# acids-ircam/RAVE

Hardware: AMD Instinct MI355X
Metric: audio samples/sec/GPU (RAVE v2 training step, 44.1 kHz, n_signal=65536) (higher is better)
Workload: dtype f32; 1 GPU; v2 config, batch 32 mono 44.1 kHz n_signal=65536, VAE-phase training step per GPU (--phase vae); global_batch=32, parallelism=dp1, phase=vae

## Files before the change

include/rave_hip.h:

```cpp
#ifndef RAVE_HIP_H
#define RAVE_HIP_H

#include <stddef.h>
#include <stdint.h>

#ifdef __cplusplus
extern "C" {
#endif

#define RH_VERSION 100

#define RH_OK 0
#define RH_ERR_INVALID (-1)
#define RH_ERR_UNSUPPORTED (-2)
#define RH_ERR_WORKSPACE (-3)

typedef void* rh_stream_t;

enum rh_act {
    RH_ACT_NONE = 0,
    RH_ACT_LEAKY = 1,
    RH_ACT_SNAKE = 2
};

// ... 21 lines not shown
const char* rh_last_error(void);



int rh_weight_norm_fwd_f32(const float* v, const float* g, int64_t rows, int64_t cols, float* w,
                           float* norms, rh_stream_t stream);
int rh_weight_norm_bwd_f32(const float* dw, const float* v, const float* g, const float* norms,
                           int64_t rows, int64_t cols, float* dv, float* dg, rh_stream_t stream);
typedef struct rh_wn_bwd_item {
    const float* dw;
    const float* v;
    const float* g;
    const float* norms;
    float* dv;
    float* dg;
    int64_t rows;
    int64_t cols;
} rh_wn_bwd_item;
int rh_weight_norm_bwd_batched_f32(const rh_wn_bwd_item* items, int32_t n_items, rh_stream_t stream);
typedef struct rh_reduce_item {
    const float* part;
    float* out;
    int64_t n;
    int32_t Z;
    int32_t reserved;
} rh_reduce_item;
int rh_defer_reduce(rh_reduce_item* item);
int rh_reduce_partials_batched_f32(const rh_reduce_item* items, int32_t n_items, rh_stream_t stream);

int64_t rh_conv1d_packed_floats(const rh_conv1d_desc* d, int which);
int rh_conv1d_pack_f32(const rh_conv1d_desc* d, const float* w, float* wp_fwd, float* wp_bwd,
                       rh_stream_t stream);

int rh_conv1d_pack_wn_f32(const rh_conv1d_desc* d, const float* v, const float* g, float* norms,
                          float* scale, float* wp_fwd, float* wp_bwd, rh_stream_t stream);

int64_t rh_prep_item_bytes(void);
int64_t rh_prep_array_bytes(int32_t n);
int rh_prep_fill_item(const rh_conv1d_desc* d, const float* v, const float* g, float* norms, float* scale,
                      float* wp_fwd, float* wp_bwd, void* item_host);
int rh_prep_link(void* items_host, int32_t n, int64_t* total_rows, int64_t* total_blocks);
int rh_prep_run_f32(const void* items_dev, int32_t n, int64_t total_rows, int64_t total_blocks, rh_stream_t stream);


int rh_conv1d_fwd_f32(const rh_conv1d_desc* d, const float* x, const float* wp_fwd,
                      const float* bias, const float* snake_alpha, const float* residual,
                      float* y, void* workspace, int64_t workspace_bytes, rh_stream_t stream);
int64_t rh_conv1d_fwd_workspace_bytes(const rh_conv1d_desc* d);
int64_t rh_conv1d_bwd_data_workspace_bytes(const rh_conv1d_desc* d);
int rh_conv1d_kernel_family(const rh_conv1d_desc* d, int which, int has_bias, int has_add);
int rh_residual_unit_fused(const rh_conv1d_desc* d3, const rh_conv1d_desc* d1);
int rh_residual_unit_fwd_f32(const rh_conv1d_desc* d3, const rh_conv1d_desc* d1, const float* x, const float* wp3_fwd,
                             const float* wp1_fwd, float* h, float* y, rh_stream_t stream);

int rh_x6_uses_ranges(void);
int rh_x6_range_words(void);
int rh_x6_set_ranges(const uint32_t* in_a, const uint32_t* in_b, uint32_t* out, uint32_t* out2);
int rh_amax_f32(const float* x, int64_t n, uint32_t* slot, rh_stream_t stream);

int rh_conv1d_plan_info(const rh_conv1d_desc* d, int which, int has_bias, int has_add, int32_t* out8);
int rh_conv1d_bwd_weight_kernel_family(const rh_conv1d_desc* d);

int rh_conv1d_bwd_data_f32(const rh_conv1d_desc* d, const float* dy, const float* wp_bwd,
                           const float* x, const float* snake_alpha, const float* add, float* dx,
                           void* workspace, int64_t workspace_bytes, rh_stream_t stream);

int64_t rh_conv1d_workspace_bytes(const rh_conv1d_desc* d);
int rh_conv1d_bwd_weight_f32(const rh_conv1d_desc* d, const float* dy, const float* x,
                             const float* snake_alpha, float* dw, float* dbias, void* workspace,
                             int64_t workspace_bytes, rh_stream_t stream);
int rh_conv1d_bwd_weight_wn_f32(const rh_conv1d_desc* d, const float* dy, const float* x, const float* snake_alpha,
                                const float* v, const float* g, const float* norms, float* dw_scratch, float* dv,
                                float* dg, float* dbias, void* workspace, int64_t workspace_bytes, rh_stream_t stream);
int64_t rh_conv1d_bwd_weight_wn_fused_launches(void);


int rh_pqmf_analysis_fwd_f32(const float* x, const float* w, int32_t rows, int32_t t_len,
                             int32_t n_band, int32_t kernel, int32_t pad_left, int32_t n_frames,
                             float* y, rh_stream_t stream);
int rh_pqmf_analysis_bwd_f32(const float* dy, const float* w, int32_t rows, int32_t t_len,
                             int32_t n_band, int32_t kernel, int32_t pad_left, int32_t n_frames,
                             float* dx, rh_stream_t stream);
int rh_pqmf_synthesis_fwd_f32(const float* y, const float* w, int32_t rows, int32_t n_frames,
                              int32_t n_band, int32_t kernel, int32_t pad_left, int32_t n_out,
                              float* x, rh_stream_t stream);
int rh_pqmf_synthesis_bwd_f32(const float* dx, const float* w, int32_t rows, int32_t n_frames,
                              int32_t n_band, int32_t kernel, int32_t pad_left, int32_t n_out,
                              float* dy, rh_stream_t stream);

int rh_pqmf_fold_k1_f32(const float* in, const float* tab, int32_t rows, int32_t t_len, int32_t n_frames, int32_t o0,
                        float scale, float* out, rh_stream_t stream);
int rh_pqmf_fold_k2_f32(const float* in, const float* tab, int32_t rows, int32_t n_frames, int32_t n_out, int32_t dp,
                        float scale, float* out, rh_stream_t stream);


int rh_amp_tanh_fwd_f32(const float* x, int32_t batch, int32_t c, int32_t l, float* y,
                        rh_stream_t stream);
int rh_amp_tanh_bwd_f32(const float* dy, const float* x, int32_t batch, int32_t c, int32_t l,
                        float* dx, rh_stream_t stream);
int rh_act_fwd_f32(const float* x, const float* snake_alpha, int32_t act, float slope,
                   int32_t batch, int32_t c, int32_t l, float* y, rh_stream_t stream);
int64_t rh_snake_bwd_workspace_bytes(int32_t batch, int32_t c);
int rh_snake_bwd_f32(const float* dy, const float* x, const float* alpha, int32_t batch, int32_t c,
                     int32_t l, float* dx, float* dalpha, void* workspace, int64_t workspace_bytes,
                     rh_stream_t stream);
int rh_act_bwd_f32(const float* dy, const float* y, int32_t act, float slope, int64_t n, float* g, rh_stream_t stream);
// ... 132 lines not shown
```

rave_amd/_lib.py:

```python
from __future__ import annotations

import ctypes as C
import os

import torch

_HERE = os.path.dirname(os.path.abspath(__file__))
LIB_PATH = os.environ.get("RAVE_HIP_LIB") or os.path.join(_HERE, "librave_hip.so")

ACT_NONE, ACT_LEAKY, ACT_SNAKE = 0, 1, 2


class ConvDesc(C.Structure):
    _fields_ = [
        ("batch", C.c_int32), ("c_in", C.c_int32), ("c_out", C.c_int32),
        ("l_in", C.c_int32), ("l_out", C.c_int32), ("kernel", C.c_int32),
        ("stride", C.c_int32), ("dilation", C.c_int32), ("pad_left", C.c_int32),
        ("transposed", C.c_int32), ("groups", C.c_int32), ("inner", C.c_int32),
        ("in_valid", C.c_int32), ("act", C.c_int32), ("act_slope", C.c_float),
        ("out_act", C.c_int32), ("out_slope", C.c_float),
    ]


class AdamItem(C.Structure):
# ... 3 lines not shown
class WnBwdItem(C.Structure):
    _fields_ = [("dw", C.c_void_p), ("v", C.c_void_p), ("g", C.c_void_p), ("norms", C.c_void_p), ("dv", C.c_void_p),
                ("dg", C.c_void_p), ("rows", C.c_int64), ("cols", C.c_int64)]


class ReduceItem(C.Structure):
    _fields_ = [("part", C.c_void_p), ("out", C.c_void_p), ("n", C.c_int64), ("Z", C.c_int32), ("reserved", C.c_int32)]


class LossItem(C.Structure):
    _fields_ = [("value", C.c_void_p), ("w1_dev", C.c_void_p), ("w1", C.c_float), ("w2", C.c_float)]


class FmItem(C.Structure):
    _fields_ = [("f", C.c_void_p), ("df", C.c_void_p), ("half", C.c_int64), ("w", C.c_float)]


class Conv2dDesc(C.Structure):
    _fields_ = [(n, C.c_int32) for n in (
        "batch", "c_in", "c_out", "h_in", "w_in", "h_out", "w_out", "kh", "kw", "sh", "sw", "dh", "dw", "ph", "pw",
        "act")] + [("act_slope", C.c_float)]


def _load() -> C.CDLL:
    if not os.path.exists(LIB_PATH):
        raise RuntimeError(
            f"rave_amd: {LIB_PATH} not found. Build it with `python -m rave_amd.build` "
            "(or __graft_entry__.build()). There is no CPU / PyTorch fallback for the HIP hot path.")
    lib = C.CDLL(LIB_PATH)
    P, I32, I64, F = C.c_void_p, C.c_int32, C.c_int64, C.c_float
    D = C.POINTER(ConvDesc)
    D2 = C.POINTER(Conv2dDesc)
    sig = {
        "rh_version": ([], C.c_int),
        "rh_last_error": ([], C.c_char_p),
        "rh_weight_norm_fwd_f32": ([P, P, I64, I64, P, P, P], C.c_int),
        "rh_weight_norm_bwd_f32": ([P, P, P, P, I64, I64, P, P, P], C.c_int),
        "rh_weight_norm_bwd_batched_f32": ([C.POINTER(WnBwdItem), I32, P], C.c_int),
        "rh_defer_reduce": ([C.POINTER(ReduceItem)], C.c_int),
        "rh_reduce_partials_batched_f32": ([C.POINTER(ReduceItem), I32, P], C.c_int),
        "rh_conv1d_packed_floats": ([D, C.c_int], I64),
        "rh_conv1d_pack_f32": ([D, P, P, P, P], C.c_int),
        "rh_conv1d_pack_wn_f32": ([D, P, P, P, P, P, P, P], C.c_int),
        "rh_prep_item_bytes": ([], I64),
        "rh_prep_array_bytes": ([I32], I64),
        "rh_prep_fill_item": ([D, P, P, P, P, P, P, P], C.c_int),
        "rh_prep_link": ([P, I32, C.POINTER(I64), C.POINTER(I64)], C.c_int),
        "rh_prep_run_f32": ([P, I32, I64, I64, P], C.c_int),
        "rh_conv1d_fwd_f32": ([D, P, P, P, P, P, P, P, I64, P], C.c_int),
        "rh_conv1d_bwd_data_f32": ([D, P, P, P, P, P, P, P, I64, P], C.c_int),
        "rh_conv1d_kernel_family": ([D, C.c_int, C.c_int, C.c_int], C.c_int),
        "rh_conv1d_bwd_weight_kernel_family": ([D], C.c_int),
        "rh_residual_unit_fused": ([D, D], C.c_int),
        "rh_residual_unit_fwd_f32": ([D, D, P, P, P, P, P, P], C.c_int),
        "rh_conv1d_plan_info": ([D, C.c_int, C.c_int, C.c_int, C.POINTER(C.c_int32)], C.c_int),
        "rh_conv1d_fwd_workspace_bytes": ([D], I64),
        "rh_conv1d_bwd_data_workspace_bytes": ([D], I64),
        "rh_conv1d_workspace_bytes": ([D], I64),
        "rh_conv1d_bwd_weight_f32": ([D, P, P, P, P, P, P, I64, P], C.c_int),
        "rh_conv1d_bwd_weight_wn_f32": ([D, P, P, P, P, P, P, P, P, P, P, P, I64, P], C.c_int),
        "rh_conv1d_bwd_weight_wn_fused_launches": ([], I64),
        "rh_conv2d_packed_floats": ([D2, C.c_int], I64),
        "rh_conv2d_pack_f32": ([D2, P, P, P, P], C.c_int),
        "rh_conv2d_fwd_f32": ([D2, P, P, P, P, P], C.c_int),
        "rh_conv2d_bwd_data_f32": ([D2, P, P, P, P, P], C.c_int),
        "rh_conv2d_workspace_bytes": ([D2], I64),
        "rh_conv2d_plan_info": ([D2, I32, C.POINTER(I64)], C.c_int),
        "rh_conv2d_bwd_weight_kernel_family": ([D2], C.c_int),
        "rh_conv2d_bwd_weight_f32": ([D2, P, P, P, P, P, P, I64, P], C.c_int),
        "rh_feed_batch_i16_f32": ([P, P, P, P, I32, I32, I32, P, P], C.c_int),
        "rh_vq_loss_partials": ([I64], I64),
        "rh_vq_assign_f32": ([P, P, I64, I32, I32, P, P, P, P, P], C.c_int),
        "rh_vq_assign_workspace_bytes": ([I64, I32, I32], I64),
        "rh_vq_assign_ws_f32": ([P, P, I64, I32, I32, P, P, P, P, P, I64, P], C.c_int),
        "rh_vq_ema_update_f32": ([P, P, I64, I32, I32, F, F, P, P, P, P], C.c_int),
        "rh_pqmf_analysis_fwd_f32": ([P, P, I32, I32, I32, I32, I32, I32, P, P], C.c_int),
        "rh_pqmf_analysis_bwd_f32": ([P, P, I32, I32, I32, I32, I32, I32, P, P], C.c_int),
        "rh_pqmf_synthesis_fwd_f32": ([P, P, I32, I32, I32, I32, I32, I32, P, P], C.c_int),
        "rh_pqmf_synthesis_bwd_f32": ([P, P, I32, I32, I32, I32, I32, I32, P, P], C.c_int),
        "rh_pqmf_fold_k1_f32": ([P, P, I32, I32, I32, I32, F, P, P], C.c_int),
        "rh_pqmf_fold_k2_f32": ([P, P, I32, I32, I32, I32, F, P, P], C.c_int),
        "rh_amp_tanh_fwd_f32": ([P, I32, I32, I32, P, P], C.c_int),
        "rh_amp_tanh_bwd_f32": ([P, P, I32, I32, I32, P, P], C.c_int),
        "rh_act_fwd_f32": ([P, P, I32, F, I32, I32, I32, P, P], C.c_int),
        "rh_act_bwd_f32": ([P, P, I32, F, I64, P, P], C.c_int),
        "rh_act_bwd_bias_workspace_bytes": ([I32], I64),
        "rh_act_bwd_bias_f32": ([P, P, I32, F, I32, I32, I64, P, P, P, I64, P], C.c_int),
        "rh_snake_bwd_workspace_bytes": ([I32, I32], I64),
        "rh_snake_bwd_f32": ([P, P, P, I32, I32, I32, P, P, P, I64, P], C.c_int),
        "rh_stft_frame_fwd_f32": ([P, P, I64, I32, I32, I32, I32, P, P], C.c_int),
        "rh_stft_frame_bwd_f32": ([P, P, I64, I32, I32, I32, I32, P, P], C.c_int),
        "rh_stft_frame_bwd_acc_f32": ([P, P, I64, I32, I32, I32, I32, P, I32, P], C.c_int),
        "rh_spectral_total_f32": ([P, P, I32, P, P], C.c_int),
        "rh_feature_matching_workspace_bytes": ([C.POINTER(FmItem), I32], I64),
        "rh_feature_matching_fwd_f32": ([C.POINTER(FmItem), I32, I32, P, I64, P, P, P], C.c_int),
        "rh_feature_matching_bwd_f32": ([C.POINTER(FmItem), I32, I32, P, P, P], C.c_int),
        "rh_reparam_workspace_bytes": ([], I64),
        "rh_reparam_fwd_f32": ([P, P, I32, I32, I32, P, P, P, I64, P], C.c_int),
        "rh_reparam_bwd_f32": ([P, P, P, P, I32, I32, I32, P, P], C.c_int),
        "rh_loss_combine_fwd_f32": ([C.POINTER(LossItem), I32, P, P, P], C.c_int),
        "rh_loss_combine_bwd_f32": ([C.POINTER(LossItem), I32, P, P, P], C.c_int),
        "rh_adam_step_f32": ([C.POINTER(AdamItem), I32, P, F, F, F, P, P], C.c_int),
        "rh_x6_uses_ranges": ([], C.c_int),
        "rh_x6_range_words": ([], C.c_int),
        "rh_x6_set_ranges": ([P, P, P, P], C.c_int),
        "rh_amax_f32": ([P, I64, P, P], C.c_int),
# ... 42 lines not shown
```

rave_amd/build.py:

```python
from __future__ import annotations

import hashlib
import os
import subprocess
import sys
from concurrent.futures import ThreadPoolExecutor

HERE = os.path.dirname(os.path.abspath(__file__))
CSRC = os.path.join(HERE, "csrc")
OBJ = os.path.join(HERE, "_obj")
LIB = os.path.join(HERE, "librave_hip.so")
SOURCES = ["api.cpp", "pqmf.hip", "pqmf_fold.hip", "pqmf_fold2.hip", "conv_igemm.hip", "conv_igemm_dma.hip", "conv_x6.hip", "conv_x6_i1_121.hip", "conv_x6_i1_221.hip", "conv_x6_i1_321.hip", "conv_x6_i1_122.hip", "conv_x6_i1_222.hip", "conv_x6_i1_322.hip", "conv_x6_i1_211.hip", "conv_x6_i1_311.hip", "conv_x6_i1_212.hip", "conv_x6_i1_312.hip", "conv_x6_i2_121.hip", "conv_x6_i2_221.hip", "conv_x6_i2_321.hip", "conv_x6_i2_122.hip", "conv_x6_i2_222.hip", "conv_x6_i2_322.hip", "conv_x6_i2_211.hip", "conv_x6_i2_311.hip", "conv_x6_i2_212.hip", "conv_x6_i2_312.hip", "conv_x6_i4_121.hip", "conv_x6_i4_221.hip", "conv_x6_i4_321.hip", "conv_x6_i4_122.hip", "conv_x6_i4_222.hip", "conv_x6_i4_322.hip", "conv_x6_i4_211.hip", "conv_x6_i4_311.hip", "conv_x6_i4_212.hip", "conv_x6_i4_312.hip", "unit_x6.hip", "conv_host.hip", "conv_wgrad.hip", "conv_wgrad_x6.hip", "conv_smallc.hip", "conv2d.hip", "conv2d_x6.hip", "conv2d_smallm.hip", "conv2d_smallc.hip", "wgrad2d_x6.hip", "vq.hip", "feed.hip", "misc.hip", "stft_loss.hip", "adam.hip", "feature_match.hip"]
HEADERS = ["common.hpp", "conv_params.hpp", "conv2d_x6.hpp", "conv_x6_kernel.inc", os.path.join("..", "..", "include", "rave_hip.h")]
FLAGS = ["--offload-arch=gfx950", "-O3", "-std=c++17", "-fPIC", "-Wall", "-Wno-unused-function"]


def _hipcc() -> str:
    for c in (os.environ.get("HIPCC"), "/opt/rocm/bin/hipcc", "hipcc"):
        if c and (os.path.isabs(c) and os.path.exists(c) or not os.path.isabs(c)):
            return c
    raise RuntimeError("hipcc not found")


def _digest(paths) -> str:
    h = hashlib.sha256()
    for p in paths:
        with open(p, "rb") as f:
            h.update(f.read())
    h.update(" ".join(FLAGS).encode())
    return h.hexdigest()


def build(force: bool = False, verbose: bool = False, _variants: bool = True) -> str:
    os.makedirs(OBJ, exist_ok=True)
    hdrs = [os.path.join(CSRC, h) for h in HEADERS]
    hip = _hipcc()
    jobs = []
    objs = []
    for s in SOURCES:
        src = os.path.join(CSRC, s)
        obj = os.path.join(OBJ, s + ".o")
        stamp = obj + ".sha"
        dig = _digest([src] + hdrs)
        objs.append(obj)
        if not force and os.path.exists(obj) and os.path.exists(stamp) and open(stamp).read() == dig:
            continue
        lang = ["-x", "hip"] if s.endswith(".hip") or s.endswith(".cpp") else []
        jobs.append((s, [hip] + FLAGS + lang + ["-c", src, "-o", obj], stamp, dig))

    def run(job):
        name, cmd, stamp, dig = job
        r = subprocess.run(cmd, capture_output=True, text=True)
        if r.returncode != 0:
            raise RuntimeError(f"hipcc failed for {name}:\n{r.stdout}\n{r.stderr}")
        if verbose and r.stderr.strip():
            print(r.stderr, file=sys.stderr)
        with open(stamp, "w") as f:
            f.write(dig)
        return name

    if jobs:
        with ThreadPoolExecutor(max_workers=min(len(jobs), os.cpu_count() or 4)) as ex:
            list(ex.map(run, jobs))
    if jobs or not os.path.exists(LIB) or force:
        cmd = [hip, "--offload-arch=gfx950", "-shared", "-fPIC", "-o", LIB] + objs
        r = subprocess.run(cmd, capture_output=True, text=True)
# ... 91 lines not shown
```

rave_amd/csrc/unit_x6.hip:

```cpp
#include <cstdlib>
#include <mutex>
#include <type_traits>
#include "conv_params.hpp"
#include "conv_x6_kernel.inc"

bool rh_conv_x6_plan_fixed(ConvP& p, int tm, int tn, int wm, size_t* lds, dim3* grid);

namespace {

struct UnitP {
    ConvP c;
    const unsigned* wq1;
    unsigned wq1_bytes;
    float slope2;
    float* h_out;
    const unsigned* w1_range;
    unsigned* h_range;
};

template <int TM, int TN>
__global__ __launch_bounds__(256, 2) void unit_x6_kernel(const UnitP u) {
    const ConvP& p = u.c;
    constexpr int WN = 4;
    constexpr int BM = 32 * TM;
    constexpr int A_UNITS = 2 * kX6P * BM;
    constexpr int NAL = (A_UNITS + 255) / 256;
    constexpr int NQ = WN * TN == 8 ? 3 : 2;
    extern __shared__ __attribute__((aligned(16))) unsigned char smem_raw[];
    u32x4* const a_st = reinterpret_cast<u32x4*>(smem_raw);
    u32x4* const b_st = a_st + 2 * A_UNITS;

    const int tid = threadIdx.x, lane = tid & 63;
    const int wn = __builtin_amdgcn_readfirstlane(tid >> 6);
    const int j = lane & 31, g = lane >> 5;

    const int tap0 = p.ph_tap0[0];
    const int minoff = p.ph_minoff[0];
    const int nu = p.ph_ntaps[0];
    const int bt = blockIdx.x / p.tiles_per_b;
    const int nt = blockIdx.x - bt * p.tiles_per_b;
    const int b0 = bt * p.nb;
    const int n0 = nt * p.bnl;
    const int pitch = p.pitch, P = p.x6_P;
    const float slope1 = p.in_act == RH_ACT_LEAKY ? p.in_slope : 1.f;

    const auto in_rsrc = __builtin_amdgcn_make_buffer_rsrc(const_cast<float*>(p.in), 0, p.in_bytes, 0x00020000);
    const auto w_rsrc = __builtin_amdgcn_make_buffer_rsrc(const_cast<unsigned*>(p.wq), 0, p.wq_bytes, 0x00020000);
#if RH_X6_F16
    int inv_x, inv_w3, inv_h, inv_w1;
    const unsigned xmax = rh_range_max(p.in_range);
    const float xsc = __uint_as_float(rh_x6_scale_bits(xmax, &inv_x));
    (void)rh_x6_scale_bits(p.w_range[0], &inv_w3);
    const float osc1 = __uint_as_float(rh_x6_unscale_bits(inv_w3, inv_x));
    const float hbound = __uint_as_float(xmax) * __uint_as_float(p.w_range[1]);
    const unsigned hsc_bits = rh_x6_scale_bits(__float_as_uint(hbound), &inv_h);
    (void)rh_x6_scale_bits(u.w1_range[0], &inv_w1);
    const float osc2 = __uint_as_float(rh_x6_unscale_bits(inv_w1, inv_h));
    const float h2sc = __uint_as_float(rh_x6_unscale_bits(inv_w3 + (int)(hsc_bits >> 23) - 127, inv_x));
#else
    const float xsc = 1.f, osc1 = 1.f, osc2 = 1.f, h2sc = 1.f;
#endif

    int bpos[TN];
#pragma unroll
    for (int tn = 0; tn < TN; ++tn) {
        const int col = (wn * TN + tn) * 32 + j;
        const int bl = col >> p.bnl_shift;
        const int nl = col & (p.bnl - 1);
        const int n = min(n0 + nl, p.ncols - 1);
        bpos[tn] = g * kX6P * P + bl * pitch + (n - n0);
    }
// ... 194 lines not shown
            for (int r = 0; r < 16; ++r) acc2[tm][0][r] = 0.f;
#pragma unroll
        for (int b = 0; b < 2 * TM; ++b) {
            const int tmh = b >> 1, hf = b & 1;
            float v[8];
#pragma unroll
            for (int i = 0; i < 8; ++i) v[i] = acc[tmh][tn][8 * hf + i];
            u32x4 pk[kX6P];
            split8(v, u.slope2, h2sc, pk);
            rh_x6_frag bfr2[kX6P], afr2[TM][kX6P];
#pragma unroll
            for (int s3 = 0; s3 < kX6P; ++s3) {
                auto r0 = __builtin_amdgcn_permlane32_swap(pk[s3][0], pk[s3][2], false, false);
                auto r1 = __builtin_amdgcn_permlane32_swap(pk[s3][1], pk[s3][3], false, false);
                u32x4 f;
                f[0] = r0[0]; f[2] = r0[1]; f[1] = r1[0]; f[3] = r1[1];
                bfr2[s3] = __builtin_bit_cast(rh_x6_frag, f);
            }
            const u32x4* al = w1s + (b * 2 * kX6P + g * kX6P) * BM + j;
#pragma unroll
            for (int tm = 0; tm < TM; ++tm)
#pragma unroll
                for (int s3 = 0; s3 < kX6P; ++s3) afr2[tm][s3] = __builtin_bit_cast(rh_x6_frag, al[s3 * BM + tm * 32]);
#pragma unroll
            for (int q = 0; q < RH_X6_NPROD; ++q)
#pragma unroll
                for (int tm = 0; tm < TM; ++tm)
                    acc2[tm][0] = RH_X6_MFMA(afr2[tm][SA[q]], bfr2[SB[q]], acc2[tm][0]);
        }
        const unsigned cb1[1] = {cb[tn]};
        x6_store_tile<4, TM, 1>(acc2, cb1, 0, g, p.M, full, p.out_row, y_r, none_r, x_r, none_r, 1.f, 0.f, osc2, ymax);
    }
    if (RH_X6_F16 && (p.out_range || u.h_range)) {
        __syncthreads();
        float* red = reinterpret_cast<float*>(smem_raw);
        if (p.out_range) rh_range_publish(p.out_range, ymax, blockIdx.x, red);
        if (u.h_range) rh_range_publish(u.h_range, hmax_all, blockIdx.x + 5u, red + 4);
    }
}

bool unit_enabled() {
    const char* e = getenv("RH_UNIT_FUSED");
    if (e && atoi(e) == 0) return false;
    const char* x6 = getenv("RH_CONV_X6");
    return !(x6 && atoi(x6) == 0);
}

bool unit_shape_ok(const rh_conv1d_desc* d3, const rh_conv1d_desc* d1) {
    if (!d3 || !d1) return false;
    const int C = d3->c_in;
    auto act_ok = [](const rh_conv1d_desc* d) {
        return d->act == RH_ACT_NONE || (d->act == RH_ACT_LEAKY && d->act_slope >= 0.f && d->act_slope <= 1.f);
    };
    return (C == 32 || C == 64 || C == 96) && d3->c_out == C && d1->c_in == C && d1->c_out == C && !d3->transposed &&
           !d1->transposed && d3->stride == 1 && d1->stride == 1 && d3->inner == 1 && d1->inner == 1 && d3->groups == 1 &&
           d1->groups == 1 && d1->kernel == 1 && d1->dilation == 1 && d1->pad_left == 0 && d3->in_valid == 0 &&
           d1->in_valid == 0 && d3->out_act == RH_ACT_NONE && d1->out_act == RH_ACT_NONE && act_ok(d3) && act_ok(d1) &&
           d3->batch > 0 && d3->batch == d1->batch && d3->l_in > 0 && d3->l_out == d3->l_in && d1->l_in == d3->l_in &&
           d1->l_out == d3->l_in;
}

int fill_unit(const rh_conv1d_desc* d3, const rh_conv1d_desc* d1, UnitP* u, size_t* lds, dim3* grid) {
    ConvP& p = u->c;
    if (int e = rh_conv_fill_fwd(d3, &p)) return e;
    ConvP p1{};
    if (int e = rh_conv_fill_fwd(d1, &p1)) return e;
    if (p.x6_mode != 1 || p1.x6_mode != 1 || p.nphase != 1) return RH_ERR_UNSUPPORTED;
    const int tm = p.M / 32;
    if (!rh_conv_x6_plan_fixed(p, tm, 2, 1, lds, grid)) return RH_ERR_UNSUPPORTED;
    const size_t w1_bytes = (size_t)(p.M / 16) * 2 * kX6P * p.M * 16;
    if (w1_bytes > *lds) *lds = w1_bytes;
    if (*lds > 160 * 1024 || (unsigned long long)p1.wq_bytes < w1_bytes) return RH_ERR_UNSUPPORTED;
    u->wq1_bytes = p1.wq_bytes;
    u->slope2 = d1->act == RH_ACT_LEAKY ? d1->act_slope : 1.f;
    u->h_out = nullptr;
    u->wq1 = reinterpret_cast<const unsigned*>((uintptr_t)p1.x6_wofs);
    return RH_OK;
}

}

extern "C" int rh_residual_unit_fused(const rh_conv1d_desc* d3, const rh_conv1d_desc* d1) {
    if (!unit_enabled() || !unit_shape_ok(d3, d1)) return 0;
    UnitP u{};
    size_t lds = 0;
    dim3 grid;
    static const unsigned any_range[kRangeSlotWords] = {};
    u.c.in_range = any_range;
    return fill_unit(d3, d1, &u, &lds, &grid) == RH_OK ? 1 : 0;
}

extern "C" int rh_residual_unit_fwd_f32(const rh_conv1d_desc* d3, const rh_conv1d_desc* d1, const float* x, const float* wp3_fwd,
                                        const float* wp1_fwd, float* h, float* y, rh_stream_t stream) {
    const RhKernelEventsScope events;
    const unsigned* x_range = nullptr;
    unsigned *y_range = nullptr, *h_range = nullptr;
    rh_take_ranges(nullptr, &x_range, &y_range, &h_range);
    RH_REQUIRE(unit_enabled() && unit_shape_ok(d3, d1), RH_ERR_UNSUPPORTED, "residual_unit_fwd: geometry not fusable");
    RH_REQUIRE(x && wp3_fwd && wp1_fwd && y, RH_ERR_INVALID, "residual_unit_fwd: null pointer");
    UnitP u{};
    size_t lds = 0;
    dim3 grid;
    RH_REQUIRE(!RH_X6_F16 || x_range, RH_ERR_INVALID, "residual_unit_fwd: the f16 kernels need the input's range slot (rh_x6_set_ranges)");
    u.c.in_range = x_range;
    if (int e = fill_unit(d3, d1, &u, &lds, &grid)) {
        rh_set_error("residual_unit_fwd: geometry not fusable");
        return e;
    }
    ConvP& p = u.c;
    p.in_range = x_range; p.out_range = y_range; u.h_range = h ? h_range : nullptr;
    RH_REQUIRE((((uintptr_t)wp3_fwd | (uintptr_t)wp1_fwd) & 15) == 0 && ((uintptr_t)x & 3) == 0, RH_ERR_INVALID,
               "residual_unit_fwd: misaligned operand");
    p.in = x; p.wp = wp3_fwd; p.out = y; p.bias = nullptr; p.add = x; p.mul_src = nullptr;
    p.wq = reinterpret_cast<const unsigned*>(wp3_fwd + p.x6_wofs);
    p.in_alpha = nullptr; p.mul_alpha = nullptr;
    p.in_bytes = (unsigned)(4ull * p.B * p.C * (unsigned long long)p.in_row);
    u.wq1 = reinterpret_cast<const unsigned*>(wp1_fwd + (long)(uintptr_t)u.wq1);
    p.w_range = p.wq + p.wq_bytes / 4;
    u.w1_range = u.wq1 + u.wq1_bytes / 4;
    u.h_out = h;
    auto go = [&](auto kern) {
        static std::once_flag once;
        std::call_once(once, [&] {
            (void)hipFuncSetAttribute(reinterpret_cast<const void*>(kern), hipFuncAttributeMaxDynamicSharedMemorySize, 160 * 1024);
        });
        rh_launch_main(kern, grid, dim3(256), lds, (hipStream_t)stream, u);
    };
    const int tm = p.M / 32;
    if (tm == 1) go(unit_x6_kernel<1, 2>);
    else if (tm == 2) go(unit_x6_kernel<2, 2>);
    else go(unit_x6_kernel<3, 2>);
    return rh_check_launch("residual_unit_fwd");
}
```

rave_amd/ops.py:

```python
from __future__ import annotations

import ctypes as C
import os
from dataclasses import dataclass
from typing import Optional, Tuple

import torch

from . import _lib as L
from ._lib import ACT_LEAKY, ACT_NONE, ACT_SNAKE

Tensor = torch.Tensor


_PROFILE = None
_EVENT_POOL = []


def profile_begin() -> None:
    global _PROFILE
    _PROFILE = []


def _hip_event():
# ... 308 lines not shown
        slot = _valid_slot(base, s)
        if slot is not None:
            t._rh_range = (slot, t._version) + tuple(base._rh_range[2:])
            return slot
    if _RANGE_MISS is not None:
        _RANGE_MISS.append((tag, tuple(t.shape)))
    slot = _new_range(t.device)
    L.check(L.lib.rh_amax_f32(L.ptr(t), t.numel(), L.ptr(slot), s), "amax")
    _attach_range(t, slot)
    side = next((st for st in _SIDE.values() if st.cuda_stream == s), None)
    if side is not None:
        ev = torch.cuda.Event()
        ev.record(side)
        t._rh_range = (slot, t._version, (s, torch.cuda.is_current_stream_capturing(), ev))
    return slot


def _fwd(d, x, wp, bias, alpha, residual, y, s):
    _log_plan(d, 0, bias is not None, residual is not None)
    ws = _ws(L.lib.rh_conv1d_fwd_workspace_bytes(C.byref(d)), y.device)
    rin = rout = None
    if _ranges_on():
        if L.lib.rh_conv1d_kernel_family(C.byref(d), 0, int(bias is not None), int(residual is not None)) == 1:
            rin = _range_of(x, s, "fwd x")
        rout = _new_range(y.device)

    @_armed_call
    def run(out, ranges=True):
        if ranges and rout is not None:
            L.lib.rh_x6_set_ranges(None, L.ptr(rin), L.ptr(rout), None)
        return L.lib.rh_conv1d_fwd_f32(C.byref(d), L.ptr(x), L.ptr(wp), L.ptr(bias), L.ptr(alpha), L.ptr(residual), L.ptr(out),
                                       L.ptr(ws), ws.numel() * 4 if ws is not None else 0, s)

    rc = _launch("conv_fwd", d, lambda: run(y), bias is not None, residual is not None)
    if rc == 0:
        _attach_range(y, rout)
        _shadow("fwd", d, lambda o: run(o[0], False), [y])
    return rc


def _unit_fwd(d3, d1, x, wp3, wp1, h, y, s):
    rin = ry = rh = None
    if _RANGES:
        rin, ry = _range_of(x, s, "unit x"), _new_range(x.device)
        rh = _new_range(x.device) if h is not None else None

    @_armed_call
    def run(o_y, o_h):
        if rin is not None:
            L.lib.rh_x6_set_ranges(None, L.ptr(rin), L.ptr(ry), L.ptr(rh))
        return L.lib.rh_residual_unit_fwd_f32(C.byref(d3), C.byref(d1), L.ptr(x), L.ptr(wp3), L.ptr(wp1), L.ptr(o_h), L.ptr(o_y), s)

    if _PLAN_LOG is not None:
        _PLAN_LOG.append((2, (d3.c_in, d3.c_out, d3.kernel, d3.stride, d3.dilation, d3.l_in, d3.transposed), (3, d3.c_in // 32, 2, 1, 1, 1, 0, 0)))
    if _PROFILE is None:
        rc = run(y, h)
    else:
        f3, b3 = _conv_cost(d3)
        f1, b1 = _conv_cost(d1)
        rc = _timed("conv_fwd[x6]", f3 + f1, b3 + b1, lambda: run(y, h))
    if rc == 0:
        _attach_range(y, ry)
        _attach_range(h, rh)
    if rc == 0 and _SHADOW is not None:
        h2, y2 = torch.empty_like(x), torch.empty_like(x)
        with _ExactF32():
            nf3 = L.lib.rh_conv1d_fwd_workspace_bytes(C.byref(d3))
            nf1 = L.lib.rh_conv1d_fwd_workspace_bytes(C.byref(d1))
            ws = _ws(max(nf3, nf1, 4), x.device)
            L.check(L.lib.rh_conv1d_fwd_f32(C.byref(d3), L.ptr(x), L.ptr(wp3), None, None, None, L.ptr(h2), L.ptr(ws), ws.numel() * 4, s),
                    "shadow unit k3")
            L.check(L.lib.rh_conv1d_fwd_f32(C.byref(d1), L.ptr(h2), L.ptr(wp1), None, None, L.ptr(x), L.ptr(y2), L.ptr(ws), ws.numel() * 4, s),
                    "shadow unit k1")
        key = (d3.c_in, d3.c_out, d3.kernel, d3.stride, d3.dilation, d3.l_in, d3.transposed, d3.batch)
        _SHADOW.append(("unit", key, _rel(y, y2)))
        if h is not None:
            _SHADOW.append(("unit_h", key, _rel(h, h2)))
    return rc


def _dgrad(d, dy, wp, x, alpha, add, dx, s):
    _log_plan(d, 1, False, add is not None)
    ws = _ws(L.lib.rh_conv1d_bwd_data_workspace_bytes(C.byref(d)), dx.device)
    rin = rout = None
    if _ranges_on():
        if L.lib.rh_conv1d_kernel_family(C.byref(d), 1, 0, int(add is not None)) == 1:
            rin = _range_of(dy, s, "dgrad dy")
        rout = _new_range(dx.device)

    @_armed_call
    def run(out, ranges=True):
        if ranges and rout is not None:
            L.lib.rh_x6_set_ranges(None, L.ptr(rin), L.ptr(rout), None)
        return L.lib.rh_conv1d_bwd_data_f32(C.byref(d), L.ptr(dy), L.ptr(wp), L.ptr(x), L.ptr(alpha), L.ptr(add), L.ptr(out),
                                            L.ptr(ws), ws.numel() * 4 if ws is not None else 0, s)

    rc = _launch("conv_dgrad", d, lambda: run(dx), False, add is not None)
    if rc == 0:
        _attach_range(dx, rout)
        _shadow("dgrad", d, lambda o: run(o[0], False), [dx])
    return rc


_SIDE = {}
_SIDE_PENDING = [None]
_SIDE_HOLD = []


def _side_enabled() -> bool:
    import os
    return os.environ.get("RH_BWD_SIDE_STREAM", "1") != "0"


def _side_stream(device):
    k = device.index if device.index is not None else torch.cuda.current_device()
    st = _SIDE.get(k)
    if st is None:
        st = _SIDE[k] = torch.cuda.Stream(device=device)
    return st


_WN_PENDING = []
import os as _os
_WN_BATCH_MAX = int(_os.environ.get("RH_WN_BATCH_MAX", "64"))


def _wn_batch_enabled() -> bool:
    import os
    return os.environ.get("RH_WN_BATCH", "1") != "0"

# ... 1208 lines not shown
```

Before: 239.8 million samples/s.

## Extend fused residual-unit kernel to 192/384 channels via LDS-staged intermediate

```diff
diff --git a/include/rave_hip.h b/include/rave_hip.h
--- a/include/rave_hip.h
+++ b/include/rave_hip.h
@@ -97,6 +97,7 @@
 int rh_residual_unit_fused(const rh_conv1d_desc* d3, const rh_conv1d_desc* d1);
 int rh_residual_unit_fwd_f32(const rh_conv1d_desc* d3, const rh_conv1d_desc* d1, const float* x, const float* wp3_fwd,
                              const float* wp1_fwd, float* h, float* y, rh_stream_t stream);
+int rh_residual_unit_plan_info(const rh_conv1d_desc* d3, const rh_conv1d_desc* d1, int32_t* out8);
 
 int rh_x6_uses_ranges(void);
 int rh_x6_range_words(void);
diff --git a/rave_amd/_lib.py b/rave_amd/_lib.py
--- a/rave_amd/_lib.py
+++ b/rave_amd/_lib.py
@@ -79,6 +79,7 @@
         "rh_conv1d_kernel_family": ([D, C.c_int, C.c_int, C.c_int], C.c_int),
         "rh_conv1d_bwd_weight_kernel_family": ([D], C.c_int),
         "rh_residual_unit_fused": ([D, D], C.c_int),
+        "rh_residual_unit_plan_info": ([D, D, C.POINTER(C.c_int32)], C.c_int),
         "rh_residual_unit_fwd_f32": ([D, D, P, P, P, P, P, P], C.c_int),
         "rh_conv1d_plan_info": ([D, C.c_int, C.c_int, C.c_int, C.POINTER(C.c_int32)], C.c_int),
         "rh_conv1d_fwd_workspace_bytes": ([D], I64),
diff --git a/rave_amd/build.py b/rave_amd/build.py
--- a/rave_amd/build.py
+++ b/rave_amd/build.py
@@ -10,8 +10,8 @@
 CSRC = os.path.join(HERE, "csrc")
 OBJ = os.path.join(HERE, "_obj")
 LIB = os.path.join(HERE, "librave_hip.so")
-SOURCES = ["api.cpp", "pqmf.hip", "pqmf_fold.hip", "pqmf_fold2.hip", "conv_igemm.hip", "conv_igemm_dma.hip", "conv_x6.hip", "conv_x6_i1_121.hip", "conv_x6_i1_221.hip", "conv_x6_i1_321.hip", "conv_x6_i1_122.hip", "conv_x6_i1_222.hip", "conv_x6_i1_322.hip", "conv_x6_i1_211.hip", "conv_x6_i1_311.hip", "conv_x6_i1_212.hip", "conv_x6_i1_312.hip", "conv_x6_i2_121.hip", "conv_x6_i2_221.hip", "conv_x6_i2_321.hip", "conv_x6_i2_122.hip", "conv_x6_i2_222.hip", "conv_x6_i2_322.hip", "conv_x6_i2_211.hip", "conv_x6_i2_311.hip", "conv_x6_i2_212.hip", "conv_x6_i2_312.hip", "conv_x6_i4_121.hip", "conv_x6_i4_221.hip", "conv_x6_i4_321.hip", "conv_x6_i4_122.hip", "conv_x6_i4_222.hip", "conv_x6_i4_322.hip", "conv_x6_i4_211.hip", "conv_x6_i4_311.hip", "conv_x6_i4_212.hip", "conv_x6_i4_312.hip", "unit_x6.hip", "conv_host.hip", "conv_wgrad.hip", "conv_wgrad_x6.hip", "conv_smallc.hip", "conv2d.hip", "conv2d_x6.hip", "conv2d_smallm.hip", "conv2d_smallc.hip", "wgrad2d_x6.hip", "vq.hip", "feed.hip", "misc.hip", "stft_loss.hip", "adam.hip", "feature_match.hip"]
-HEADERS = ["common.hpp", "conv_params.hpp", "conv2d_x6.hpp", "conv_x6_kernel.inc", os.path.join("..", "..", "include", "rave_hip.h")]
+SOURCES = ["api.cpp", "pqmf.hip", "pqmf_fold.hip", "pqmf_fold2.hip", "conv_igemm.hip", "conv_igemm_dma.hip", "conv_x6.hip", "conv_x6_i1_121.hip", "conv_x6_i1_221.hip", "conv_x6_i1_321.hip", "conv_x6_i1_122.hip", "conv_x6_i1_222.hip", "conv_x6_i1_322.hip", "conv_x6_i1_211.hip", "conv_x6_i1_311.hip", "conv_x6_i1_212.hip", "conv_x6_i1_312.hip", "conv_x6_i2_121.hip", "conv_x6_i2_221.hip", "conv_x6_i2_321.hip", "conv_x6_i2_122.hip", "conv_x6_i2_222.hip", "conv_x6_i2_322.hip", "conv_x6_i2_211.hip", "conv_x6_i2_311.hip", "conv_x6_i2_212.hip", "conv_x6_i2_312.hip", "conv_x6_i4_121.hip", "conv_x6_i4_221.hip", "conv_x6_i4_321.hip", "conv_x6_i4_122.hip", "conv_x6_i4_222.hip", "conv_x6_i4_322.hip", "conv_x6_i4_211.hip", "conv_x6_i4_311.hip", "conv_x6_i4_212.hip", "conv_x6_i4_312.hip", "unit_x6.hip", "unit_lds_x6.hip", "conv_host.hip", "conv_wgrad.hip", "conv_wgrad_x6.hip", "conv_smallc.hip", "conv2d.hip", "conv2d_x6.hip", "conv2d_smallm.hip", "conv2d_smallc.hip", "wgrad2d_x6.hip", "vq.hip", "feed.hip", "misc.hip", "stft_loss.hip", "adam.hip", "feature_match.hip"]
+HEADERS = ["common.hpp", "conv_params.hpp", "conv2d_x6.hpp", "unit_x6.hpp", "conv_x6_kernel.inc", os.path.join("..", "..", "include", "rave_hip.h")]
 FLAGS = ["--offload-arch=gfx950", "-O3", "-std=c++17", "-fPIC", "-Wall", "-Wno-unused-function"]
 
 
diff --git a/rave_amd/csrc/unit_lds_x6.hip b/rave_amd/csrc/unit_lds_x6.hip
--- /dev/null
+++ b/rave_amd/csrc/unit_lds_x6.hip
@@ -0,0 +1,323 @@
+#include <cstdlib>
+#include <mutex>
+#include <type_traits>
+#include "unit_x6.hpp"
+#include "conv_x6_kernel.inc"
+
+namespace {
+
+constexpr int kTM = 3;
+
+template <int WM, int WN>
+__global__ __launch_bounds__(256, (WM == 2 ? 2 : 1)) void unit_lds_x6_kernel(const UnitP u) {
+    static_assert(WM * WN == 4, "four waves");
+    const ConvP& p = u.c;
+    constexpr int TM = kTM;
+    constexpr int BM = 32 * TM * WM;
+    constexpr int BN = 32 * WN;
+    constexpr int A_UNITS = 2 * kX6P * BM;
+    constexpr int NAL = (A_UNITS + 255) / 256;
+    constexpr int NQ = 2;
+    extern __shared__ __attribute__((aligned(16))) unsigned char smem_raw[];
+    u32x4* const a_st = reinterpret_cast<u32x4*>(smem_raw);
+    u32x4* const b_st = a_st + 2 * A_UNITS;
+
+    const int tid = threadIdx.x, lane = tid & 63;
+    const int wave = __builtin_amdgcn_readfirstlane(tid >> 6);
+    const int wm = wave / WN, wn = wave - wm * WN;
+    const int j = lane & 31, g = lane >> 5;
+
+    const int tap0 = p.ph_tap0[0];
+    const int minoff = p.ph_minoff[0];
+    const int nu = p.ph_ntaps[0];
+    const int bt = blockIdx.x / p.tiles_per_b;
+    const int nt = blockIdx.x - bt * p.tiles_per_b;
+    const int b0 = bt * p.nb;
+    const int n0 = nt * p.bnl;
+    const int pitch = p.pitch, P = p.x6_P;
+    const float slope1 = p.in_act == RH_ACT_LEAKY ? p.in_slope : 1.f;
+
+    const auto in_rsrc = __builtin_amdgcn_make_buffer_rsrc(const_cast<float*>(p.in), 0, p.in_bytes, 0x00020000);
+    const auto w_rsrc = __builtin_amdgcn_make_buffer_rsrc(const_cast<unsigned*>(p.wq), 0, p.wq_bytes, 0x00020000);
+    const auto w1_rsrc = __builtin_amdgcn_make_buffer_rsrc(const_cast<unsigned*>(u.wq1), 0, u.wq1_bytes, 0x00020000);
+#if RH_X6_F16
+    int inv_x, inv_w3, inv_h, inv_w1;
+    const unsigned xmax = rh_range_max(p.in_range);
+    const float xsc = __uint_as_float(rh_x6_scale_bits(xmax, &inv_x));
+    (void)rh_x6_scale_bits(p.w_range[0], &inv_w3);
+    const float osc1 = __uint_as_float(rh_x6_unscale_bits(inv_w3, inv_x));
+    const float hbound = __uint_as_float(xmax) * __uint_as_float(p.w_range[1]);
+    const unsigned hsc_bits = rh_x6_scale_bits(__float_as_uint(hbound), &inv_h);
+    (void)rh_x6_scale_bits(u.w1_range[0], &inv_w1);
+    const float osc2 = __uint_as_float(rh_x6_unscale_bits(inv_w1, inv_h));
+    const float h2sc = __uint_as_float(rh_x6_unscale_bits(inv_w3 + (int)(hsc_bits >> 23) - 127, inv_x));
+#else
+    const float xsc = 1.f, osc1 = 1.f, osc2 = 1.f, h2sc = 1.f;
+#endif
+
+    const int col = wn * 32 + j;
+    int bpos;
+    {
+        const int bl = col >> p.bnl_shift;
+        const int nl = col & (p.bnl - 1);
+        const int n = min(n0 + nl, p.ncols - 1);
+        bpos = g * kX6P * P + bl * pitch + (n - n0);
+    }
+    const int arow = g * kX6P * BM + wm * TM * 32 + j;
+
+    f32x16 acc[TM][1];
+#pragma unroll
+    for (int tm = 0; tm < TM; ++tm)
+#pragma unroll
+        for (int r = 0; r < 16; ++r) acc[tm][0][r] = 0.f;
+
+    unsigned aoff[NAL];
+#pragma unroll
+    for (int r = 0; r < NAL; ++r) {
+        const int uu = tid + 256 * r;
+        const int gs = uu / BM, mrow = uu - gs * BM;
+        aoff[r] = (uu < A_UNITS && mrow < p.Mp) ? (unsigned)((gs * p.Mp + mrow) * 16) : kOOB;
+    }
+    const unsigned step_bytes = (unsigned)(2 * kX6P * p.Mp * 16);
+    unsigned xoff[NQ];
+    int xdst[NQ];
+#pragma unroll
+    for (int q = 0; q < NQ; ++q) {
+        const int e = tid + 256 * q;
+        const int o = e >= P ? 1 : 0;
+        const int pp = e - o * P;
+        const int bl = pp / pitch, qq = pp - bl * pitch;
+        const bool task = e < 2 * P;
+        const bool bok = task && b0 + bl < p.B;
+        xdst[q] = task ? o * kX6P * P + pp : -1;
+        const int f = n0 + minoff + qq;
+        const bool ok = bok && f >= 0 && f < p.in_valid;
+        xoff[q] = ok ? (unsigned)((((b0 + bl) * p.C + 8 * o) * p.in_row + f) * 4) : kOOB;
+    }
+    const unsigned chunk_bytes = (unsigned)(16 * p.in_row * 4);
+    unsigned rowc[8];
+#pragma unroll
+    for (int i = 0; i < 8; ++i) rowc[i] = (unsigned)(i * p.in_row * 4);
+
+    float xr[NQ][8];
+    u32x4 ar[NAL];
+    auto load_x = [&](int chunk) {
+        const unsigned cbv = (unsigned)chunk * chunk_bytes;
+#pragma unroll
+        for (int q = 0; q < NQ; ++q)
+#pragma unroll
+            for (int i = 0; i < 8; ++i)
+                xr[q][i] = __builtin_bit_cast(float, __builtin_amdgcn_raw_buffer_load_b32(in_rsrc, xoff[q], cbv + rowc[i], 0));
+    };
+    auto split = [&](const auto& v, float slope, float sc, unsigned (&pk)[kX6P][4]) {
+        constexpr int N = sizeof(v) / sizeof(float);
+#if RH_X6_F16
+#pragma unroll
+        for (int k = 0; k < N / 2; ++k) {
+            float a = v[2 * k] * sc, b = v[2 * k + 1] * sc;
+            a = rh_max1(a, a * slope);
+            b = rh_max1(b, b * slope);
+            const rh_h2 h = rh_h2_split(a, b);
+            pk[0][k] = h.hi; pk[1][k] = h.lo;
+        }
+#else
+        unsigned h[3][N];
+#pragma unroll
+        for (int i = 0; i < N; ++i) {
+            const float a = rh_max1(v[i], v[i] * slope);
+            rh_bf3_split(a, h[0][i], h[1][i], h[2][i]);
+        }
+#pragma unroll
+        for (int s3 = 0; s3 < 3; ++s3)
+#pragma unroll
+            for (int k = 0; k < N / 2; ++k) pk[s3][k] = __builtin_amdgcn_perm(h[s3][2 * k + 1], h[s3][2 * k], 0x07060302u);
+#endif
+    };
+    auto convert_x = [&](int stage) {
+        u32x4* dst0 = b_st + stage * 2 * kX6P * P;
+#pragma unroll
+        for (int q = 0; q < NQ; ++q) {
+            if (xdst[q] < 0) continue;
+            unsigned pk[kX6P][4];
+            split(xr[q], slope1, xsc, pk);
+#pragma unroll
+            for (int s3 = 0; s3 < kX6P; ++s3) dst0[xdst[q] + s3 * P] = u32x4{pk[s3][0], pk[s3][1], pk[s3][2], pk[s3][3]};
+        }
+    };
+    const int nchunks = p.C >> 4;
+    const int S = nchunks * nu;
+    const unsigned sbytes0 = (unsigned)(p.ph_q2ofs[0] * 16);
+    auto load_a = [&](__amdgpu_buffer_rsrc_t rs, unsigned base, int step) {
+        const unsigned sb = base + (unsigned)step * step_bytes;
+#pragma unroll
+        for (int r = 0; r < NAL; ++r) {
+            if (r * 256 >= A_UNITS) continue;
+            ar[r] = __builtin_bit_cast(u32x4, __builtin_amdgcn_raw_buffer_load_b128(rs, aoff[r], sb, 0));
+        }
+    };
+    auto store_a = [&](int stage) {
+#pragma unroll
+        for (int r = 0; r < NAL; ++r) {
+            const int uu = tid + 256 * r;
+            if (uu < A_UNITS) a_st[stage * A_UNITS + uu] = ar[r];
+        }
+    };
+    constexpr int SA[RH_X6_NPROD] = RH_X6_SA, SB[RH_X6_NPROD] = RH_X6_SB;
+
+    load_a(w_rsrc, sbytes0, 0);
+    load_x(0);
+    store_a(0);
+    if (S > 1) load_a(w_rsrc, sbytes0, 1);
+    convert_x(0);
+    if (nchunks > 1) load_x(1);
+    __syncthreads();
+    int st = 0;
+    int toff_next = p.off[tap0] - minoff;
+    for (int ci = 0; ci < nchunks; ++ci) {
+        const u32x4* bl_ = b_st + (ci & 1) * 2 * kX6P * P;
+        for (int t = 0; t < nu; ++t, ++st) {
+            const int toff = toff_next;
+            {
+                const int t1 = t + 1 < nu ? t + 1 : 0;
+                toff_next = p.off[tap0 + t1] - minoff;
+            }
+            const u32x4* al = a_st + (st & 1) * A_UNITS + arow;
+            rh_x6_frag bfr[kX6P], afr[TM][kX6P];
+#pragma unroll
+            for (int s3 = 0; s3 < kX6P; ++s3) bfr[s3] = __builtin_bit_cast(rh_x6_frag, bl_[bpos + s3 * P + toff]);
+#pragma unroll
+            for (int tm = 0; tm < TM; ++tm)
+#pragma unroll
+                for (int s3 = 0; s3 < kX6P; ++s3) afr[tm][s3] = __builtin_bit_cast(rh_x6_frag, al[s3 * BM + tm * 32]);
+            if (st + 1 < S) {
+                store_a((st + 1) & 1);
+                if (st + 2 < S) load_a(w_rsrc, sbytes0, st + 2);
+            }
+            if (t == nu - 1 && ci + 1 < nchunks) {
+                convert_x((ci + 1) & 1);
+                if (ci + 2 < nchunks) load_x(ci + 2);
+            }
+#pragma unroll
+            for (int q = 0; q < RH_X6_NPROD; ++q)
+#pragma unroll
+                for (int tm = 0; tm < TM; ++tm) acc[tm][0] = RH_X6_MFMA(afr[tm][SA[q]], bfr[SB[q]], acc[tm][0]);
+            __syncthreads();
+        }
+    }
+
+    const int S2 = nchunks;
+    load_a(w1_rsrc, 0u, 0);
+
+    unsigned cb[1];
+    {
+        const int bl = col >> p.bnl_shift;
+        const int nl = col & (p.bnl - 1);
+        const int n = n0 + nl, b = b0 + bl;
+        const bool ok = n < p.ncols && b < p.B && n < p.out_valid;
+        cb[0] = ok ? (unsigned)(((long)b * p.M * p.out_row + n) * 4) : kOOB;
+    }
+    const unsigned obytes = (unsigned)(p.part_stride * 4);
+    const auto y_r = __builtin_amdgcn_make_buffer_rsrc(p.out, 0, obytes, 0x00020000);
+    const auto x_r = __builtin_amdgcn_make_buffer_rsrc(const_cast<float*>(p.add), 0, obytes, 0x00020000);
+    const auto none_r = __builtin_amdgcn_make_buffer_rsrc(static_cast<float*>(nullptr), 0, 0, 0x00020000);
+    const int mrow0 = wm * TM * 32;
+    float hmax_all = 0.f;
+    if (u.h_out) {
+        const auto h_r = __builtin_amdgcn_make_buffer_rsrc(u.h_out, 0, obytes, 0x00020000);
+        x6_store_tile<0, TM, 1>(acc, cb, mrow0, g, p.M, true, p.out_row, h_r, none_r, none_r, none_r, 1.f, 0.f, osc1, hmax_all);
+    }
+
+    {
+        unsigned char* img = reinterpret_cast<unsigned char*>(b_st);
+#pragma unroll
+        for (int tm = 0; tm < TM; ++tm)
+#pragma unroll
+            for (int q = 0; q < 4; ++q) {
+                float v[4];
+#pragma unroll
+                for (int i = 0; i < 4; ++i) v[i] = acc[tm][0][4 * q + i];
+                unsigned pk[kX6P][4];
+                split(v, u.slope2, h2sc, pk);
+                const int chunk = (mrow0 + 32 * tm) / 16 + (q >> 1);
+                const int unit0 = ((chunk * 2 + (q & 1)) * kX6P) * BN + col;
+#pragma unroll
+                for (int s3 = 0; s3 < kX6P; ++s3) {
+                    typedef unsigned u32x2 __attribute__((ext_vector_type(2)));
+                    *reinterpret_cast<u32x2*>(img + (size_t)(unit0 + s3 * BN) * 16 + 8 * g) = u32x2{pk[s3][0], pk[s3][1]};
+                }
+            }
+    }
+#pragma unroll
+    for (int tm = 0; tm < TM; ++tm)
+#pragma unroll
+        for (int r = 0; r < 16; ++r) acc[tm][0][r] = 0.f;
+    store_a(0);
+    if (S2 > 1) load_a(w1_rsrc, 0u, 1);
+    __syncthreads();
+
+    {
+        const u32x4* hb = b_st + g * kX6P * BN + col;
+        for (int s = 0; s < S2; ++s) {
+            const u32x4* al = a_st + (s & 1) * A_UNITS + arow;
+            const u32x4* bl_ = hb + s * 2 * kX6P * BN;
+            rh_x6_frag bfr[kX6P], afr[TM][kX6P];
+#pragma unroll
+            for (int s3 = 0; s3 < kX6P; ++s3) bfr[s3] = __builtin_bit_cast(rh_x6_frag, bl_[s3 * BN]);
+#pragma unroll
+            for (int tm = 0; tm < TM; ++tm)
+#pragma unroll
+                for (int s3 = 0; s3 < kX6P; ++s3) afr[tm][s3] = __builtin_bit_cast(rh_x6_frag, al[s3 * BM + tm * 32]);
+            if (s + 1 < S2) {
+                store_a((s + 1) & 1);
+                if (s + 2 < S2) load_a(w1_rsrc, 0u, s + 2);
+            }
+#pragma unroll
+            for (int q = 0; q < RH_X6_NPROD; ++q)
+#pragma unroll
+                for (int tm = 0; tm < TM; ++tm) acc[tm][0] = RH_X6_MFMA(afr[tm][SA[q]], bfr[SB[q]], acc[tm][0]);
+            __syncthreads();
+        }
+    }
+    float ymax = 0.f;
+    x6_store_tile<4, TM, 1>(acc, cb, mrow0, g, p.M, true, p.out_row, y_r, none_r, x_r, none_r, 1.f, 0.f, osc2, ymax);
+    if (RH_X6_F16 && (p.out_range || u.h_range)) {
+        float* red = reinterpret_cast<float*>(smem_raw);
+        if (p.out_range) rh_range_publish(p.out_range, ymax, blockIdx.x, red);
+        if (u.h_range) rh_range_publish(u.h_range, hmax_all, blockIdx.x + 5u, red + 4);
+    }
+}
+
+}
+
+static int unit_lds_level() {
+    const char* e = getenv("RH_UNIT_LDS");
+    return e ? atoi(e) : 1;
+}
+bool rh_unit_lds_enabled() { return unit_lds_level() > 0; }
+
+bool rh_unit_lds_plan(UnitP& u, size_t* lds, dim3* grid) {
+    ConvP& p = u.c;
+    if (!rh_unit_lds_enabled() || (p.M != 192 && p.M != 384) || p.Mp != p.M || p.C != p.M) return false;
+    if (p.M == 384 && unit_lds_level() < 2) return false;
+    const int wm = p.M / (32 * kTM);
+    size_t lds1 = 0;
+    if (!rh_conv_x6_plan_fixed(p, kTM, 1, wm, &lds1, grid)) return false;
+    const int bn = 32 * (4 / wm);
+    const size_t a_bytes = (size_t)2 * p.x6_a_units * 16;
+    const size_t image = (size_t)(p.M / 16) * 2 * kX6P * bn * 16;
+    const size_t b_bytes = (size_t)2 * p.x6_b_units * 16;
+    *lds = a_bytes + (image > b_bytes ? image : b_bytes);
+    return *lds <= (size_t)160 * 1024;
+}
+
+void rh_unit_lds_launch(const UnitP& u, dim3 grid, size_t lds, hipStream_t stream) {
+    auto go = [&](auto kern) {
+        static std::once_flag once;
+        std::call_once(once, [&] {
+            (void)hipFuncSetAttribute(reinterpret_cast<const void*>(kern), hipFuncAttributeMaxDynamicSharedMemorySize, 160 * 1024);
+        });
+        rh_launch_main(kern, grid, dim3(256), lds, stream, u);
+    };
+    if (u.c.M == 192) go(unit_lds_x6_kernel<2, 2>);
+    else go(unit_lds_x6_kernel<4, 1>);
+}
diff --git a/rave_amd/csrc/unit_x6.hip b/rave_amd/csrc/unit_x6.hip
--- a/rave_amd/csrc/unit_x6.hip
+++ b/rave_amd/csrc/unit_x6.hip
@@ -1,22 +1,10 @@
 #include <cstdlib>
 #include <mutex>
 #include <type_traits>
-#include "conv_params.hpp"
+#include "unit_x6.hpp"
 #include "conv_x6_kernel.inc"
 
-bool rh_conv_x6_plan_fixed(ConvP& p, int tm, int tn, int wm, size_t* lds, dim3* grid);
-
 namespace {
-
-struct UnitP {
-    ConvP c;
-    const unsigned* wq1;
-    unsigned wq1_bytes;
-    float slope2;
-    float* h_out;
-    const unsigned* w1_range;
-    unsigned* h_range;
-};
 
 template <int TM, int TN>
 __global__ __launch_bounds__(256, 2) void unit_x6_kernel(const UnitP u) {
@@ -317,7 +305,7 @@
     auto act_ok = [](const rh_conv1d_desc* d) {
         return d->act == RH_ACT_NONE || (d->act == RH_ACT_LEAKY && d->act_slope >= 0.f && d->act_slope <= 1.f);
     };
-    return (C == 32 || C == 64 || C == 96) && d3->c_out == C && d1->c_in == C && d1->c_out == C && !d3->transposed &&
+    return (C == 32 || C == 64 || C == 96 || C == 192 || C == 384) && d3->c_out == C && d1->c_in == C && d1->c_out == C && !d3->transposed &&
            !d1->transposed && d3->stride == 1 && d1->stride == 1 && d3->inner == 1 && d1->inner == 1 && d3->groups == 1 &&
            d1->groups == 1 && d1->kernel == 1 && d1->dilation == 1 && d1->pad_left == 0 && d3->in_valid == 0 &&
            d1->in_valid == 0 && d3->out_act == RH_ACT_NONE && d1->out_act == RH_ACT_NONE && act_ok(d3) && act_ok(d1) &&
@@ -331,11 +319,15 @@
     ConvP p1{};
     if (int e = rh_conv_fill_fwd(d1, &p1)) return e;
     if (p.x6_mode != 1 || p1.x6_mode != 1 || p.nphase != 1) return RH_ERR_UNSUPPORTED;
-    const int tm = p.M / 32;
-    if (!rh_conv_x6_plan_fixed(p, tm, 2, 1, lds, grid)) return RH_ERR_UNSUPPORTED;
     const size_t w1_bytes = (size_t)(p.M / 16) * 2 * kX6P * p.M * 16;
-    if (w1_bytes > *lds) *lds = w1_bytes;
-    if (*lds > 160 * 1024 || (unsigned long long)p1.wq_bytes < w1_bytes) return RH_ERR_UNSUPPORTED;
+    if (p.M > 96) {
+        if (!rh_unit_lds_plan(*u, lds, grid) || (unsigned long long)p1.wq_bytes < w1_bytes) return RH_ERR_UNSUPPORTED;
+    } else {
+        const int tm = p.M / 32;
+        if (!rh_conv_x6_plan_fixed(p, tm, 2, 1, lds, grid)) return RH_ERR_UNSUPPORTED;
+        if (w1_bytes > *lds) *lds = w1_bytes;
+        if (*lds > 160 * 1024 || (unsigned long long)p1.wq_bytes < w1_bytes) return RH_ERR_UNSUPPORTED;
+    }
     u->wq1_bytes = p1.wq_bytes;
     u->slope2 = d1->act == RH_ACT_LEAKY ? d1->act_slope : 1.f;
     u->h_out = nullptr;
@@ -353,6 +345,22 @@
     static const unsigned any_range[kRangeSlotWords] = {};
     u.c.in_range = any_range;
     return fill_unit(d3, d1, &u, &lds, &grid) == RH_OK ? 1 : 0;
+}
+
+extern "C" int rh_residual_unit_plan_info(const rh_conv1d_desc* d3, const rh_conv1d_desc* d1, int32_t* out8) {
+    RH_REQUIRE(out8, RH_ERR_INVALID, "residual_unit_plan_info: null output");
+    for (int i = 0; i < 8; ++i) out8[i] = 0;
+    if (!unit_enabled() || !unit_shape_ok(d3, d1)) return RH_OK;
+    UnitP u{};
+    size_t lds = 0;
+    dim3 grid;
+    static const unsigned any_range[kRangeSlotWords] = {};
+    u.c.in_range = any_range;
+    if (fill_unit(d3, d1, &u, &lds, &grid) != RH_OK) return RH_OK;
+    const bool wide = u.c.M > 96;
+    out8[0] = 3; out8[1] = wide ? 3 : u.c.M / 32; out8[2] = wide ? 1 : 2; out8[3] = wide ? u.c.M / 96 : 1;
+    out8[4] = 1; out8[5] = 1; out8[6] = 0; out8[7] = (int32_t)grid.x;
+    return RH_OK;
 }
 
 extern "C" int rh_residual_unit_fwd_f32(const rh_conv1d_desc* d3, const rh_conv1d_desc* d1, const float* x, const float* wp3_fwd,
@@ -392,7 +400,8 @@
         rh_launch_main(kern, grid, dim3(256), lds, (hipStream_t)stream, u);
     };
     const int tm = p.M / 32;
-    if (tm == 1) go(unit_x6_kernel<1, 2>);
+    if (tm > 3) rh_unit_lds_launch(u, grid, lds, (hipStream_t)stream);
+    else if (tm == 1) go(unit_x6_kernel<1, 2>);
     else if (tm == 2) go(unit_x6_kernel<2, 2>);
     else go(unit_x6_kernel<3, 2>);
     return rh_check_launch("residual_unit_fwd");
diff --git a/rave_amd/csrc/unit_x6.hpp b/rave_amd/csrc/unit_x6.hpp
--- /dev/null
+++ b/rave_amd/csrc/unit_x6.hpp
@@ -0,0 +1,18 @@
+#pragma once
+#include "conv_params.hpp"
+
+struct UnitP {
+    ConvP c;
+    const unsigned* wq1;
+    unsigned wq1_bytes;
+    float slope2;
+    float* h_out;
+    const unsigned* w1_range;
+    unsigned* h_range;
+};
+
+bool rh_conv_x6_plan_fixed(ConvP& p, int tm, int tn, int wm, size_t* lds, dim3* grid);
+
+bool rh_unit_lds_enabled();
+bool rh_unit_lds_plan(UnitP& u, size_t* lds, dim3* grid);
+void rh_unit_lds_launch(const UnitP& u, dim3 grid, size_t lds, hipStream_t stream);
diff --git a/rave_amd/ops.py b/rave_amd/ops.py
--- a/rave_amd/ops.py
+++ b/rave_amd/ops.py
@@ -384,7 +384,9 @@
         return L.lib.rh_residual_unit_fwd_f32(C.byref(d3), C.byref(d1), L.ptr(x), L.ptr(wp3), L.ptr(wp1), L.ptr(o_h), L.ptr(o_y), s)
 
     if _PLAN_LOG is not None:
-        _PLAN_LOG.append((2, (d3.c_in, d3.c_out, d3.kernel, d3.stride, d3.dilation, d3.l_in, d3.transposed), (3, d3.c_in // 32, 2, 1, 1, 1, 0, 0)))
+        out = (C.c_int32 * 8)()
+        L.check(L.lib.rh_residual_unit_plan_info(C.byref(d3), C.byref(d1), out), "residual_unit_plan_info")
+        _PLAN_LOG.append((2, (d3.c_in, d3.c_out, d3.kernel, d3.stride, d3.dilation, d3.l_in, d3.transposed), tuple(out)))
     if _PROFILE is None:
         rc = run(y, h)
     else:
@@ -405,9 +407,17 @@
             L.check(L.lib.rh_conv1d_fwd_f32(C.byref(d1), L.ptr(h2), L.ptr(wp1), None, None, L.ptr(x), L.ptr(y2), L.ptr(ws), ws.numel() * 4, s),
                     "shadow unit k1")
         key = (d3.c_in, d3.c_out, d3.kernel, d3.stride, d3.dilation, d3.l_in, d3.transposed, d3.batch)
-        _SHADOW.append(("unit", key, _rel(y, y2)))
-        if h is not None:
-            _SHADOW.append(("unit_h", key, _rel(h, h2)))
+        if d3.c_in <= 96:
+            _SHADOW.append(("unit", key, _rel(y, y2)))
+            if h is not None:
+                _SHADOW.append(("unit_h", key, _rel(h, h2)))
+        else:
+            if h is not None:
+                _SHADOW.append(("fwd", key, _rel(h, h2)))
+                with _ExactF32():
+                    L.check(L.lib.rh_conv1d_fwd_f32(C.byref(d1), L.ptr(h), L.ptr(wp1), None, None, L.ptr(x), L.ptr(y2), L.ptr(ws),
+                                                    ws.numel() * 4, s), "shadow unit k1")
+            _SHADOW.append(("fwd", (d1.c_in, d1.c_out, d1.kernel, d1.stride, d1.dilation, d1.l_in, d1.transposed, d1.batch), _rel(y, y2)))
     return rc
 
 
```

Result: no change. 241.4 million samples/s (median of 6 runs) (+0.6%).
